# awslabs/palace

Hardware: AMD Instinct MI355X
Metric: curl-curl Mult DOF/s + PCG iters/s, p=3 H(curl) 10M DOF @1/2/4/8 GPU (higher is better)
Workload: dtype f64

## Files before the change

palace_amd/csrc/pa_internal.hpp:

```cpp
#pragma once

#include <hip/hip_runtime.h>

#include <cstdint>
#include <cstdio>
#include <stdexcept>
#include <string>
#include <vector>

#include "../../include/palace_amd.h"
#include "pa_stream_host.hpp"

struct pa_op;
typedef struct pa_op pa_op_fwd;

struct pa_csr {
  bool symmetric = true;
  int32_t nrows = 0;
  int32_t ncols = 0;
  int64_t nnz = 0;
  int32_t *d_rowptr = nullptr, *d_col = nullptr;
  double *d_val = nullptr;
};

// ... 128 lines not shown
  int32_t *d_lidx = nullptr;
  int32_t *d_sidx = nullptr;
  int32_t *d_sidx_bc = nullptr;
  uint16_t *d_perm = nullptr;
  uint16_t *d_perm_x = nullptr;
  int32_t *d_shared = nullptr;
  int32_t *d_shared_bc = nullptr;
  std::vector<int32_t> h_shared;
  std::vector<char> h_price_skip;
  int n_shared = 0;
  std::vector<uint16_t> h_perm;
  std::vector<int32_t> h_sidx;
  double *d_ye = nullptr;
  double *d_ye2 = nullptr;
  int32_t *d_tptr = nullptr;
  int32_t *d_tent = nullptr;
  uint32_t *d_idxc = nullptr;
  bool stream_default = true;
  uint32_t *d_perm_s_bc = nullptr;
  std::vector<uint32_t> h_perm_s;
  int32_t *d_rhdr_bc = nullptr, *d_rpos_bc = nullptr;
  int n_shared_bc = 0;
  uint32_t *d_perm_s = nullptr;
  uint32_t *d_flagw = nullptr, *d_flagw_bc = nullptr, *d_slots = nullptr;
  int n_slot_patterns = 0;
  double *d_coef_s = nullptr;
  int32_t *d_rhdr = nullptr, *d_rpos = nullptr;
  int n_runs = 0, n_runs_bc = 0;
  uint32_t *d_rchunk = nullptr, *d_rchunk_bc = nullptr;
  uint32_t *d_flagw_all = nullptr, *d_rchunk_all = nullptr;
  uint32_t *d_perm_s_all = nullptr;
  int32_t *d_rhdr_all = nullptr, *d_rpos_all = nullptr;
  int n_all = 0, n_runs_all = 0;
  std::vector<char> h_ess_flag;
  std::vector<double> Bc, Gc, Bo;
  double *d_tab = nullptr;
  bool iso = false;
  std::vector<uint8_t> ctx_blob;
  CoeffHost c0, c1;
};

struct DenseSub {
  Geom *geom = nullptr;
  int fe_type = 0, P = 0, Q = 0, Qpad = 0, nch = 0, ne = 0, nb = 0, lsize = 0, KP = 0, PT = 0;
  int qf = 0, mode = 0;
  bool contra = false;
  bool ye_rows = false;
// ... 187 lines not shown
```

palace_amd/csrc/pa_nd_hex_stream.hip:

```cpp
#include <algorithm>
#include <map>

#include "pa_nd_hex_core.hpp"

#ifndef PA_CPLX_QAHEAD
#define PA_CPLX_QAHEAD 0
#endif
#ifndef PA_STREAM_QAHEAD
#define PA_STREAM_QAHEAD 0
#endif
#ifndef PA_KM_MINW_LOW
#define PA_KM_MINW_LOW 2
#endif
#ifndef PA_KM_MINW
#define PA_KM_MINW 2
#endif

namespace pa {

typedef double d2v __attribute__((ext_vector_type(2)));

#ifdef PA_STREAM_TRACE
constexpr int kTraceWG = 64, kTraceBatches = 14, kTraceStamps = 12;
__device__ unsigned long long g_trace[kTraceWG * kTraceBatches * kTraceStamps];
#define PA_STAMP(k)                                                                                          \
  do {                                                                                                       \
    if (tr_on && tr_b < kTraceBatches && lane == 0)                                                          \
      g_trace[((size_t)blockIdx.x * kTraceBatches + tr_b) * kTraceStamps + (k)] = __builtin_readcyclecounter(); \
  } while (0)
#else
#define PA_STAMP(k) \
  do {              \
  } while (0)
#endif

#ifdef PA_STREAM_OLD_LDS
__host__ __device__ constexpr int stream_lds_elem(const int raw) { return raw; }
#else
__host__ __device__ constexpr int stream_lds_elem(const int raw) { return (raw + 15) / 32 * 32 + 16; }
#endif

template <int P1>
struct NDStreamArgs {
  int ne, nbatch, chunk;
  const uint32_t *idxc;
  const uint32_t *flagw;
  const uint32_t *slots;
  const double *qdata;
  const double *qaff;
  double wq2[2];
  const double *coef;
  const double *xn, *gtab;
  const double *x;
  double *y, *ye;
  const double *x1, *coef1;
  double *y1, *ye1;
  const double *qdata1;
  int qm[2], qc[2], qn[2];
  int nsplit;
  const double *xg0, *xg1;
  const unsigned long long *xg_sel;
  double *yg;
  NDTab<P1, 4> tab;
};

template <int P1, bool USE_U, bool USE_C, bool METRIC, int MINW, int GPOS, bool CPLX = false, bool SPLIT = false, int GEOMN = 0>
__global__ __launch_bounds__(64 * kWavesPerBlock, MINW) void nd_hex_stream_kernel(const NDStreamArgs<P1> a) {
  static_assert(!CPLX || (USE_U && USE_C), "the complex form is built on the curl-curl + mass kernels");
  static_assert(!(CPLX && SPLIT), "no split-vector form of the complex kernel");
  static_assert(!GEOMN || (!USE_U && USE_C && !METRIC && !CPLX), "geometry from the nodes: the curl-curl kernel");
  constexpr int Q1 = 4;
  constexpr bool AFF = (!CPLX || METRIC) && !GEOMN && !(PA_STREAM_QAHEAD && MINW == 2);
#ifdef PA_STREAM_EARLY
  constexpr bool EARLY_IDX = true;
#else
  constexpr bool EARLY_IDX = P1 < 3;
#endif
  using L = typename std::conditional<P1 == 3 && !CPLX && USE_C && !USE_U, NDLayoutInPlaceSwz3, NDLayout<P1, Q1>>::type;
  constexpr int NC = P1 + 1, PP = 3 * P1 * NC * NC, NPL = (PP + 15) / 16, NPK = (NPL + 3) / 4;
#ifdef PA_METRIC6
  constexpr int NG = METRIC ? 6 : 6 * ((USE_U ? 1 : 0) + (USE_C ? 1 : 0));
#else
  constexpr int NG = METRIC ? (USE_U ? 7 : 6) : 6 * ((USE_U ? 1 : 0) + (USE_C ? 1 : 0));
#endif
  static_assert(PP <= 256, "8-bit slots");
  using streamhost::kIdxPattern;
  using streamhost::kIdxStart0;
  using streamhost::kIdxWords;
  constexpr int LDS_SIDE = (PP + 1) / 2 + (NPK + 1) * 8;
  constexpr int LDS_XN = GEOMN ? 82 : 0;
  constexpr int LDS_ELEM = stream_lds_elem(L::ELEM_PAD + LDS_SIDE + 12 + LDS_XN);
  extern __shared__ __attribute__((aligned(16))) double smem[];
  const int lane = threadIdx.x & 63;
  const int wave = __builtin_amdgcn_readfirstlane(threadIdx.x >> 6);
  const int xcd = blockIdx.x & 7;
  const int base = xcd * a.chunk, bend = min(base + a.chunk, a.nbatch);
  const int stride = (int)(gridDim.x >> 3) * kWavesPerBlock;
  int b = base + (int)(blockIdx.x >> 3) * kWavesPerBlock + wave;
  if (b >= bend) return;
  const double *xsel = (CPLX && ((lane >> 4) & 1)) ? a.x1 : a.x;
  const double *xgh = nullptr;
  if (SPLIT) xgh = ((a.xg_sel ? *a.xg_sel : 0ull) & 1ull) ? a.xg1 : a.xg0;
  auto load_idx = [&](const int bb, const int sub, const int t, int (&s)[NPL + 2], unsigned (&p)[NPK + 1]) {
    const int e = CPLX ? bb * 2 + (sub >> 1) : bb * 4 + sub;
    const uint32_t *ic = a.idxc + (size_t)e * kIdxWords;
#pragma unroll
    for (int r = 0; r < NPL; r++) s[r] = (int)__builtin_nontemporal_load(&ic[r]);
    s[NPL] = (int)__builtin_nontemporal_load(&ic[kIdxStart0 + t]);
    s[NPL + 1] = (int)__builtin_nontemporal_load(&ic[kIdxStart0 + 16 + (t & 3)]);
    p[NPK] = __builtin_nontemporal_load(&a.flagw[(size_t)e * 16 + t]);
    p[0] = __builtin_nontemporal_load(&ic[kIdxPattern]);
  };
  auto gather = [&](int (&s)[NPL + 2], unsigned (&p)[NPK + 1], double (&xv)[NPL], int *stab, const int t) {
    stab[t] = s[NPL];
    if (t < 4) stab[16 + t] = s[NPL + 1];
    wave_sync();
    const unsigned fw = p[NPK];
    {
      const uint32_t *sl = a.slots + (size_t)p[0] * (NPK * 16) + t;
#pragma unroll
      for (int k = 0; k < NPK; k++) p[k] = sl[16 * k];
    }
#pragma unroll
    for (int r = 0; r < NPL; r++) {
      const unsigned w = (unsigned)s[r], low = (w & 0xffffu) & ((2u << t) - 1u);
      const int rid = (int)((w >> 16) & 31u) + __popc(low) - 1;
      const int pos = low ? 16 * r + 31 - __clz((int)low) : (int)((w >> 21) & 255u);
      int dof = stab[rid] + (t + 16 * r - pos);
      if (!(16 * r + 15 < PP) && t + 16 * r >= PP) dof = 0;
      xv[r] = SPLIT ? (dof < a.nsplit ? xsel : xgh)[dof] : xsel[dof];
      const int word = dof | ((fw >> (2 * r + 1)) & 1u ? kExclBit : 0) | ((fw >> (18 + r)) & 1u ? kEssBit : 0);
      s[r] = (fw >> (2 * r)) & 1u ? -1 - word : word;
    }
  };
  auto settle = [&](unsigned (&p)[NPK + 1]) { asm volatile("" : "+v"(p[NPK])); };
  int sA[NPL + 2];
  unsigned pA[NPK + 1];
  double xv[NPL];
  load_idx(b, lane >> 4, lane & 15, sA, pA);
  gather(sA, pA, xv,
         reinterpret_cast<int *>(smem + (size_t)(wave * 4 + (lane >> 4)) * LDS_ELEM + L::ELEM_PAD + LDS_SIDE), lane & 15);
#pragma unroll
  for (int r = 0; r < NPL; r++) asm volatile("" : "+v"(xv[r]));
  settle(pA);

  constexpr bool QAHEAD = PA_STREAM_QAHEAD && MINW == 2 && (!CPLX || (PA_CPLX_QAHEAD && !METRIC));
  d2v gq[GEOMN ? 1 : 2 * NG];
  double xl[GEOMN ? 6 : 1];
  auto load_xn = [&](const int ee, const int t) {
    const double *xp = a.xn + (size_t)ee * 81;
#pragma unroll
    for (int r = 0; r < (GEOMN ? 6 : 1); r++) xl[r] = (t + 16 * r < 81) ? __builtin_nontemporal_load(&xp[t + 16 * r]) : 0.0;
  };
  auto load_q = [&](const int ee, const int t, const int aff) {
    if (GEOMN) return load_xn(ee, t);
    if (AFF && !(CPLX && !METRIC)) {
      constexpr int NS = METRIC ? 7 : NG;
      const int rs = aff ? 1 : 16;
      const d2v *g = aff ? reinterpret_cast<const d2v *>(a.qaff) + (size_t)ee * (2 * NS)
                         : reinterpret_cast<const d2v *>(a.qdata) + ((size_t)ee * (2 * NS * 16) + t);
#pragma unroll
      for (int k = 0; k < 2 * NG; k++) gq[k] = __builtin_nontemporal_load(&g[rs * k]);
      return;
    }
    if (CPLX && !METRIC) {
      const int grp = (lane >> 4) & 1;
      const int mo = a.qm[grp], co = a.qc[grp];
// ... 23 lines not shown
    PA_STAMP(0);
    int lo = lane;
    asm volatile("" : "+v"(lo));
    const int sub = lo >> 4, t = lo & 15, ta = t & 3, tb = t >> 2;
    double *sm = smem + (size_t)(wave * 4 + sub) * LDS_ELEM;
    int *side = reinterpret_cast<int *>(sm + L::ELEM_PAD);
    int *stab = side + 2 * LDS_SIDE;
#ifdef PA_STREAM_OLD_LDS
    const int lx = L::parity_xor(sub);
#else
    constexpr int lx = 0;
#endif
    const int e = CPLX ? b * 2 + (sub >> 1) : b * 4 + sub;

    const int aff = AFF ? __builtin_amdgcn_readfirstlane((int)(pA[NPK] >> 31)) : 0;
    if (!QAHEAD) load_q(e, t, aff);
    d2v ce = {0.0, 0.0}, ci = {0.0, 0.0};
    if (METRIC || GEOMN) ce = reinterpret_cast<const d2v *>(a.coef)[e];
    if (CPLX && METRIC) ci = reinterpret_cast<const d2v *>(a.coef1)[e];

#pragma unroll
    for (int r = 0; r < NPL; r++) {
      if (16 * r + 15 < PP || t + 16 * r < PP) {
        const int sv = sA[r], df = sv >= 0 ? sv : -1 - sv;
        const double v = (df & kEssBit) ? 0.0 : xv[r];
        sm[(pA[r >> 2] >> (8 * (r & 3))) & 255u] = sv >= 0 ? v : -v;
        side[t + 16 * r] = sv;
      }
    }
#pragma unroll
    for (int k = 0; k <= NPK; k++) side[2 * ((PP + 1) / 2) + 16 * k + t] = (int)pA[k];
    PA_STAMP(1);
    wave_sync();
    double uin[3][NC];
#pragma unroll
    for (int C = 0; C < 3; C++) {
      const int ni = (C == 0) ? P1 : NC, nj = (C == 1) ? P1 : NC, nk = (C == 2) ? P1 : NC;
      const bool act = ta < nj && tb < nk;
#pragma unroll
      for (int i = 0; i < NC; i++) uin[C][i] = (act && i < ni) ? sm[C * P1 * NC * NC + i + ni * (ta + nj * tb)] : 0.0;
    }
    wave_sync();

    const int kn = b + stride;
    const bool more = kn < bend;
    const int bn = more ? kn : b;
    int sB[NPL + 2];
    unsigned pB[NPK + 1];
    if (EARLY_IDX) {
      load_idx(bn, sub, t, sB, pB);
      __builtin_amdgcn_sched_barrier(0);
    }
    PA_STAMP(2);
    double U[3][Q1], CU[3][Q1];
#pragma unroll
    for (int c = 0; c < 3; c++)
#pragma unroll
      for (int q = 0; q < Q1; q++) U[c][q] = 0.0, CU[c][q] = 0.0;
    nd_fwd_comp<0, P1, Q1, USE_U, USE_C, L>(a, e, true, true, ta, tb, lx, sm, uin[0], U, CU);
    nd_fwd_comp<1, P1, Q1, USE_U, USE_C, L>(a, e, true, true, ta, tb, lx, sm, uin[1], U, CU);
    nd_fwd_comp<2, P1, Q1, USE_U, USE_C, L>(a, e, true, true, ta, tb, lx, sm, uin[2], U, CU);

    PA_STAMP(3);
    PA_STAMP(4);
    if (!EARLY_IDX) {
      __builtin_amdgcn_sched_barrier(0);
      load_idx(bn, sub, t, sB, pB);
      __builtin_amdgcn_sched_barrier(0);
    }

    constexpr bool PARK = GEOMN == 2;
    double Pz[GEOMN ? 3 : 1][3][PARK ? 1 : 3];
    double Pl = 0.0;
    double cw = 0.0;
    double *xs = sm + L::ELEM_PAD + LDS_SIDE + 12;
    auto park = [&](const int q) -> double * { return (q < 12 ? sm + 16 * q : xs + 16 * (q - 12)) + t; };
    if (GEOMN) {
#pragma unroll
      for (int r = 0; r < 6; r++)
        if (t + 16 * r < 81) xs[t + 16 * r] = xl[r];
      wave_sync();
      const double *gt = a.gtab;
      double bx[3], gx[3], by[3], gy[3];
#pragma unroll
      for (int i = 0; i < 3; i++) bx[i] = gt[ta * 3 + i], gx[i] = gt[12 + ta * 3 + i], by[i] = gt[tb * 3 + i], gy[i] = gt[12 + tb * 3 + i];
      cw = ce[1] * gt[24 + ta] * gt[24 + tb];
#pragma unroll
      for (int k = 0; k < 3; k++) {
        double acc[3][3];
#pragma unroll
// ... 132 lines not shown
        if (AFF) {
#pragma unroll
          for (int c = 0; c < 3; c++) {
            if (USE_U) U[c][qz] *= wab;
            if (USE_C) CU[c][qz] *= wab;
          }
        }
      }
    }

    if (GEOMN == 2) wave_sync();
    PA_STAMP(5);

    if (QAHEAD) {
      __builtin_amdgcn_sched_barrier(0);
      load_q(CPLX ? bn * 2 + (sub >> 1) : bn * 4 + sub, t, 0);
      __builtin_amdgcn_sched_barrier(0);
    }
    double xB[NPL];
    nd_bwd_comp<0, P1, Q1, USE_U, USE_C, L>(a, e, true, true, ta, tb, lx, sm, uin[0], U, CU);
    PA_STAMP(6);
    if (GPOS == 1) {
      __builtin_amdgcn_sched_barrier(0);
      gather(sB, pB, xB, stab, t);
      settle(pB);
      __builtin_amdgcn_sched_barrier(0);
    }
    PA_STAMP(7);
    nd_bwd_comp<1, P1, Q1, USE_U, USE_C, L>(a, e, true, true, ta, tb, lx, sm, uin[1], U, CU);
    if (GPOS == 2) {
      __builtin_amdgcn_sched_barrier(0);
      gather(sB, pB, xB, stab, t);
      settle(pB);
      __builtin_amdgcn_sched_barrier(0);
    }
    nd_bwd_comp<2, P1, Q1, USE_U, USE_C, L>(a, e, true, true, ta, tb, lx, sm, uin[2], U, CU);

    PA_STAMP(8);
#pragma unroll
    for (int C = 0; C < 3; C++) {
      const int ni = (C == 0) ? P1 : NC, nj = (C == 1) ? P1 : NC, nk = (C == 2) ? P1 : NC;
      const bool act = ta < nj && tb < nk;
#pragma unroll
      for (int i = 0; i < NC; i++)
        if (act && i < ni) sm[C * P1 * NC * NC + i + ni * (ta + nj * tb)] = uin[C][i];
    }
    wave_sync();
#pragma unroll
    for (int r = 0; r < NPL; r++) {
      const int m = (16 * r + 15 < PP) ? t + 16 * r : min(t + 16 * r, PP - 1), mt = m & 15, mr = m >> 4;
      const unsigned fl = (unsigned)side[2 * ((PP + 1) / 2) + 16 * NPK + mt] >> (2 * mr);
      const double v = sm[((unsigned)side[2 * ((PP + 1) / 2) + 16 * (mr >> 2) + mt] >> (8 * (mr & 3))) & 255u];
      const int sv = side[m], df = sv >= 0 ? sv : -1 - sv, d = df & (kExclBit - 1);
      double *yd = (CPLX && (sub & 1)) ? a.y1 : a.y;
      if (SPLIT) yd = d < a.nsplit ? a.y : a.yg;
      double *dst = (fl & 2u) ? yd + d : ((CPLX && (sub & 1)) ? a.ye1 : a.ye) + ((size_t)e * PP + m);
      *dst = (fl & 1u) ? -v : v;
    }
    wave_sync();
    PA_STAMP(9);
#ifdef PA_STREAM_TRACE
    tr_b++;
#endif
    if (!more) break;
    b = bn;
#pragma unroll
    for (int r = 0; r < NPL; r++) sA[r] = sB[r], xv[r] = xB[r];
#pragma unroll
    for (int k = 0; k <= NPK; k++) pA[k] = pB[k];
  }
}

using streamhost::RunHdr;
using streamhost::RunChunk;

constexpr int kGatherILP = 4;
struct GatherPart2 {
  const double *ye1, *x1;
  double *y1;
};
template <bool STEP, bool DUAL = false>
__global__ __launch_bounds__(256) void et_run_gather_kernel_t(const int n, const RunChunk *__restrict__ chunk,
                                                              const RunHdr *__restrict__ hdr, const int32_t *__restrict__ rpos,
                                                              const double *__restrict__ ye, double *__restrict__ y,
                                                              const int accumulate, const double *__restrict__ x,
                                                              const int ess_policy, const int nsplit, double *__restrict__ yg,
                                                              const GatherStep st, const GatherPart2 p2) {
  const int k0 = blockIdx.x * (256 * kGatherILP) + threadIdx.x;
  const int lane = threadIdx.x & 63;
  RunHdr h[kGatherILP];
  int pe[kGatherILP], d[kGatherILP], j[kGatherILP], run[kGatherILP];
  bool live[kGatherILP], fix[kGatherILP];
// ... 242 lines not shown
      const size_t e = k / P;
      const int m = (int)(k - e * P), t = m & 15, r = m >> 4;
      pp[(e * (npk + 1) + npk) * 16 + t] |= 2u << (2 * r);
      dropped += so.h_price_skip[k] ? 1 : 0, freed += so.h_price_skip[k] ? 0 : 1;
    }
    std::vector<int32_t> shared2;
    for (int d = 0; d < so.lsize; d++)
      if (cnt2[d] > 1) shared2.push_back(d);
    fprintf(stderr, "PALACE_AMD_PRICE_BLOCK=%d: %zu of %zu E-vector entries dropped, %zu more leave the gather; shared dofs %zu -> %zu\n",
            price_group, dropped, nnz, freed, so.h_shared.size(), shared2.size());
    so.h_shared = shared2;
    so.n_shared = (int)shared2.size();
  }
  if (so.fe_type == PA_FE_HCURL && !wide_form(so)) {
    stream_affine_setup(so);
    const int npl = (P + 15) / 16, npk = (npl + 3) / 4;
    for (size_t b = 0; b < so.qd->batch_aff.size(); b++)
      if (so.qd->batch_aff[b])
        for (size_t e = 4 * b; e < 4 * b + 4; e++)
          for (int t = 0; t < 16; t++) pp[(e * (npk + 1) + npk) * 16 + t] |= streamhost::kAffBit;
  }
  so.h_perm_s = pp;
  if (so.fe_type == PA_FE_HCURL && !wide_form(so)) {
    const int npl = (P + 15) / 16, npk = (npl + 3) / 4, nep = (ne + 3) & ~3, sw = npk * 16;
    std::vector<uint32_t> flagw((size_t)nep * 16), slots;
    std::map<std::vector<uint32_t>, uint32_t> dict;
    std::vector<uint32_t> key((size_t)sw);
    for (int e = 0; e < nep; e++) {
      const uint32_t *row = &pp[(size_t)e * (npk + 1) * 16];
      std::copy(row + sw, row + sw + 16, flagw.begin() + (size_t)e * 16);
      key.assign(row, row + sw);
      auto it = dict.find(key);
      if (it == dict.end()) {
        it = dict.emplace(key, (uint32_t)dict.size()).first;
        slots.insert(slots.end(), key.begin(), key.end());
      }
      ic[(size_t)e * streamhost::kIdxWords + streamhost::kIdxPattern] = it->second;
    }
    so.n_slot_patterns = (int)dict.size();
    so.d_flagw = dev_upload(flagw.data(), flagw.size());
    so.d_slots = dev_upload(slots.data(), slots.size());
  }
  so.d_idxc = dev_upload(ic.data(), ic.size());
  so.d_perm_s = dev_upload(pp.data(), pp.size());
  if (so.qd->metric || (so.iso && so.qf == PA_QF_HDIV_33 && so.geom->d_xnodes)) stream_element_coefficients(so);

  std::vector<uint32_t> code;
  std::vector<RunHdr> hdr;
  std::vector<int32_t> rpos;
  streamhost::build_runs(ne, P, so.lsize, so.h_sidx.data(), so.h_shared, code, hdr, rpos, nullptr,
                         so.h_price_skip.empty() ? nullptr : so.h_price_skip.data());
  {
    const std::vector<RunChunk> ch = streamhost::run_chunks(code);
    so.d_rchunk = dev_upload(reinterpret_cast<const uint32_t *>(ch.data()), 4 * ch.size());
  }
  so.d_rhdr = dev_upload(reinterpret_cast<const int32_t *>(hdr.data()), 2 * hdr.size());
  so.d_rpos = dev_upload(rpos.data(), rpos.size());
  so.n_runs = (int)hdr.size() - 1;
}

void stream_set_essential(SubOp &so, const std::vector<char> &flag) {
  if (!so.d_idxc) return;
  so.h_ess_flag = flag;
  if (so.n_all > 0) {
// ... 6 lines not shown
  const bool wide = wide_form(so);
  const int npkw = ((P + 31) / 32 + 1) / 2;
  for (size_t k = 0; k < nnz; k++) {
    if (flag[streamhost::dof_of(so.h_sidx[k])]) {
      const size_t e = k / P;
      if (wide) {
        const int m = (int)(k - e * P), t = m & 31, r = m >> 5;
        uint32_t &w = pb[(e * npkw + (r >> 1)) * 32 + t];
        w &= ~(streamhost::kWideExcl << (16 * (r & 1)));
        w |= streamhost::kWideEss << (16 * (r & 1));
        continue;
      }
      const int m = (int)(k - e * P), t = m & 15, r = m >> 4;
      uint32_t &fw = pb[(e * (npk + 1) + npk) * 16 + t];
      fw &= ~(2u << (2 * r));
      fw |= 1u << (18 + r);
    }
  }
  hipFree(so.d_perm_s_bc);
  so.d_perm_s_bc = dev_upload(pb.data(), pb.size());
  if (so.d_flagw) {
    const int nep = (so.ne + 3) & ~3;
    std::vector<uint32_t> fb((size_t)nep * 16);
    for (int e = 0; e < nep; e++) std::copy(&pb[((size_t)e * (npk + 1) + npk) * 16], &pb[((size_t)e * (npk + 1) + npk) * 16] + 16, fb.begin() + (size_t)e * 16);
    hipFree(so.d_flagw_bc);
    so.d_flagw_bc = dev_upload(fb.data(), fb.size());
  }
  std::vector<int32_t> count((size_t)so.lsize, 0);
  for (size_t k = 0; k < nnz; k++) count[streamhost::dof_of(so.h_sidx[k])]++;
  std::vector<int32_t> shared;
  shared.reserve(so.h_shared.size());
  if (!so.h_price_skip.empty()) {
    std::fill(count.begin(), count.end(), 0);
    for (size_t k = 0; k < nnz; k++)
      if (!so.h_price_skip[k]) count[streamhost::dof_of(so.h_sidx[k])]++;
  }
  for (int d = 0; d < so.lsize; d++)
    if (count[d] != 1 || flag[d]) shared.push_back(d);
  std::vector<uint32_t> code;
  std::vector<RunHdr> hdr;
  std::vector<int32_t> rpos;
  streamhost::build_runs(so.ne, P, so.lsize, so.h_sidx.data(), shared, code, hdr, rpos, flag.data(),
                         so.h_price_skip.empty() ? nullptr : so.h_price_skip.data());
  hipFree(so.d_rhdr_bc), hipFree(so.d_rpos_bc), hipFree(so.d_rchunk_bc);
  {
    const std::vector<RunChunk> ch = streamhost::run_chunks(code);
    so.d_rchunk_bc = dev_upload(reinterpret_cast<const uint32_t *>(ch.data()), 4 * ch.size());
  }
  so.d_rhdr_bc = dev_upload(reinterpret_cast<const int32_t *>(hdr.data()), 2 * hdr.size());
  so.d_rpos_bc = dev_upload(rpos.data(), rpos.size());
  so.n_shared_bc = (int)shared.size();
  so.n_runs_bc = (int)hdr.size() - 1;
}

void free_stream(SubOp &so) {
  hipFree(so.d_idxc), hipFree(so.d_perm_s), hipFree(so.d_perm_s_bc), hipFree(so.d_coef_s);
  hipFree(so.d_flagw), hipFree(so.d_flagw_bc), hipFree(so.d_slots);
  hipFree(so.d_flagw_all), hipFree(so.d_perm_s_all), hipFree(so.d_rchunk_all), hipFree(so.d_rhdr_all), hipFree(so.d_rpos_all);
  so.d_flagw_all = so.d_perm_s_all = nullptr, so.d_rchunk_all = nullptr, so.d_rhdr_all = so.d_rpos_all = nullptr, so.n_all = 0;
  hipFree(so.d_rhdr), hipFree(so.d_rpos), hipFree(so.d_rhdr_bc), hipFree(so.d_rpos_bc), hipFree(so.d_rchunk), hipFree(so.d_rchunk_bc);
}

static int device_cus() {
  static int cus = [] {
    int dev = 0, n = 0;
    if (hipGetDevice(&dev) != hipSuccess || hipDeviceGetAttribute(&n, hipDeviceAttributeMultiprocessorCount, dev) != hipSuccess || n <= 0)
      n = 256;
    return n;
  }();
  return cus;
}

template <int P1, bool U, bool C, bool METRIC, int MINW, int GPOS, bool CPLX = false, bool SPLIT = false, int GEOMN = 0>
static void launch_gpos(const SubOp &so, NDStreamArgs<P1> &a, hipStream_t s) {
  using L = typename std::conditional<P1 == 3 && !CPLX && C && !U, NDLayoutInPlaceSwz3, NDLayout<P1, 4>>::type;
  for (int i = 0; i < HalfTab<P1, 4>::LEN; i++) a.tab.Bo[i] = so.Bo[i];
  for (int i = 0; i < HalfTab<P1 + 1, 4>::LEN; i++) a.tab.Bc[i] = so.Bc[i], a.tab.Gc[i] = so.Gc[i];
  constexpr int PP = 3 * P1 * (P1 + 1) * (P1 + 1);
  constexpr int NPK = ((PP + 15) / 16 + 3) / 4;
  const size_t lds = sizeof(double) * (size_t)(kWavesPerBlock * 4) *
                     stream_lds_elem(L::ELEM_PAD + (PP + 1) / 2 + (NPK + 1) * 8 + 12 + (GEOMN ? 82 : 0));
  static const int wg_env = getenv("PALACE_AMD_STREAM_WG") ? atoi(getenv("PALACE_AMD_STREAM_WG")) : 0;
  static const int per_cu_query = [&] {
    int nb = 0;
    if (hipOccupancyMaxActiveBlocksPerMultiprocessor(&nb, nd_hex_stream_kernel<P1, U, C, METRIC, MINW, GPOS, CPLX, SPLIT, GEOMN>,
                                                     64 * kWavesPerBlock, lds) != hipSuccess || nb <= 0)
      nb = 8;
    return std::min({nb, MINW * 4 / kWavesPerBlock, (int)(160 * 1024 / lds), 8});
  }();
  const int per_cu = wg_env > 0 ? wg_env : per_cu_query;
  const int per_xcd = std::max(1, device_cus() / 8) * per_cu;
  if (CPLX) a.nbatch = (so.ne + 1) / 2;
  else a.nbatch = (so.ne + 3) / 4;
  if (a.nbatch == 0) return;
  a.chunk = (a.nbatch + 7) / 8;
  const int waves = std::min(per_xcd * kWavesPerBlock, a.chunk);
  const int wgx = std::max(1, (waves + kWavesPerBlock - 1) / kWavesPerBlock);
  hipLaunchKernelGGL((nd_hex_stream_kernel<P1, U, C, METRIC, MINW, GPOS, CPLX, SPLIT, GEOMN>), dim3(8 * wgx), dim3(64 * kWavesPerBlock),
                     lds, s, a);
  PA_HIP(hipGetLastError());
}

template <int P1, bool U, bool C, bool METRIC, int MINW_>
static void launch_variant(const SubOp &so, NDStreamArgs<P1> &a, hipStream_t s) {
#ifdef PA_STREAM_MINW2
  constexpr int MINW = 2;
#else
  constexpr int MINW = MINW_;
#endif
  constexpr int GPOS = U ? 2 : 1;
  if (a.nsplit >= 0)
    return launch_gpos<P1, U, C, METRIC, MINW, GPOS, false, true>(so, a, s);
  launch_gpos<P1, U, C, METRIC, MINW, GPOS>(so, a, s);
}

template <int P1>
static void launch_p(const SubOp &so, const double *x, double *y, bool masked, hipStream_t s, const SplitIO *split,
                     bool all = false) {
  NDStreamArgs<P1> a{};
  a.nsplit = -1, a.xg0 = a.xg1 = nullptr, a.xg_sel = nullptr, a.yg = nullptr;
  if (split) {
    PA_REQUIRE(split->n_true >= 0 && split->n_true <= so.lsize, "split point outside the local vector");
    a.nsplit = split->n_true;
    a.xg0 = split->xg0 - split->n_true, a.xg1 = (split->xg1 ? split->xg1 : split->xg0) - split->n_true;
    a.xg_sel = split->sel, a.yg = split->yg - split->n_true;
  }
  a.ne = so.ne, a.nbatch = 0;
  a.idxc = so.d_idxc;
  a.flagw = all ? so.d_flagw_all : (masked ? so.d_flagw_bc : so.d_flagw);
  a.slots = so.d_slots;
  a.qdata = so.qd->d;
  a.qaff = so.qd->d_aff, a.wq2[0] = so.qd->wq2[0], a.wq2[1] = so.qd->wq2[1];
#ifdef PA_METRIC6
  if (so.geom->w1.size() == 4) a.wq2[0] = so.geom->w1[0], a.wq2[1] = so.geom->w1[1];
#endif
  a.coef = so.d_coef_s;
  a.xn = nullptr, a.gtab = nullptr;
  a.x = x, a.y = y, a.ye = so.d_ye;
  const bool m = so.qd->metric;
  switch (so.qf) {
    case PA_QF_HDIV_33: {
      const char *ge = getenv("PALACE_AMD_STREAM_GEOM");
      const bool geomn = ge && std::string(ge) == "nodes";
      if (!m && geomn && P1 == 3 && so.iso && so.geom->d_xnodes && so.d_coef_s && !split) {
        a.xn = so.geom->d_xnodes, a.gtab = so.geom->d_gtab;
        const char *ve = getenv("PALACE_AMD_GEOMN_VARIANT");
        if (ve && std::string(ve) == "w2g2") launch_gpos<P1, false, true, false, 2, 2, false, false, (P1 == 3 ? 1 : 0)>(so, a, s);
        else if (ve && std::string(ve) == "park3g1") launch_gpos<P1, false, true, false, 3, 1, false, false, (P1 == 3 ? 2 : 0)>(so, a, s);
        else if (ve && std::string(ve) == "park3g2") launch_gpos<P1, false, true, false, 3, 2, false, false, (P1 == 3 ? 2 : 0)>(so, a, s);
        else launch_gpos<P1, false, true, false, 2, 1, false, false, (P1 == 3 ? 1 : 0)>(so, a, s);
        break;
      }
      if (m) launch_variant<P1, false, true, true, (P1 == 3 ? 2 : 3)>(so, a, s); else launch_variant<P1, false, true, false, 3>(so, a, s);
// ... 43 lines not shown
  };
  if (!enabled || !qf_ok(sr) || !qf_ok(si)) return false;
  if (sr.geom != si.geom || sr.ne != si.ne || sr.p != si.p || sr.P != si.P || sr.q1d != si.q1d) return false;
  auto iso_ok = [](const SubOp &so) {
    return so.iso && ((so.q1d == 4 && so.p <= 3) || (so.q1d == 5 && so.p <= 4 && nd_hex_stream5_ok(so))) && !so.geom->h_attr.empty();
  };
  const bool metric = iso_ok(sr) && iso_ok(si) && sr.d_idxc && sr.d_coef_s && sr.qd && sr.qd->metric;
  auto packed_ok = [](const SubOp &so) {
    return ((so.q1d == 4 && so.p <= 3) || (so.q1d == 5 && so.p <= 4 && nd_hex_stream5_ok(so))) && so.qd && !so.qd->metric &&
           so.qd->ncomp == (so.qf == PA_QF_HDIVMASS_33 ? 12 : 6);
  };
  const bool packed = packed_ok(sr) && packed_ok(si) && sr.d_idxc;
  if (!metric && !packed) return false;
  return sr.h_sidx == si.h_sidx;
}

template <int P1>
static void launch_complex_p(const SubOp &sr, const SubOp &si, const double *xr, const double *xi, double *yr, double *yi,
                             double *ye_i, bool masked, hipStream_t s) {
  NDStreamArgs<P1> a{};
  a.ne = sr.ne, a.nbatch = 0;
  a.idxc = sr.d_idxc;
  a.flagw = masked ? sr.d_flagw_bc : sr.d_flagw;
  a.slots = sr.d_slots;
  a.qdata = sr.qd->d;
  if (sr.qd->metric) a.qaff = sr.qd->d_aff, a.wq2[0] = sr.qd->wq2[0], a.wq2[1] = sr.qd->wq2[1];
  a.coef = sr.d_coef_s, a.coef1 = si.d_coef_s;
  a.xn = nullptr, a.gtab = nullptr;
  a.x = xr, a.x1 = xi, a.y = yr, a.y1 = yi, a.ye = sr.d_ye, a.ye1 = ye_i;
  a.nsplit = -1, a.xg0 = a.xg1 = nullptr, a.xg_sel = nullptr, a.yg = nullptr;
  a.qdata1 = nullptr;
  if (sr.qd->metric) return launch_gpos<P1, true, true, true, 2, 2, true>(sr, a, s);
  const SubOp *ops[2] = {&sr, &si};
  for (int g = 0; g < 2; g++) {
    const int qf = ops[g]->qf;
    a.qn[g] = ops[g]->qd->ncomp;
    a.qm[g] = (qf == PA_QF_HCURL_33 || qf == PA_QF_HDIVMASS_33) ? 0 : -1;
    a.qc[g] = qf == PA_QF_HDIV_33 ? 0 : (qf == PA_QF_HDIVMASS_33 ? 6 : -1);
  }
  a.qdata1 = si.qd->d;
  launch_gpos<P1, true, true, false, 2, 2, true>(sr, a, s);
}

void launch_nd_hex_stream_complex(const SubOp &sr, const SubOp &si, const double *xr, const double *xi, double *yr, double *yi,
                                  double *ye_i, bool masked, hipStream_t s) {
  if (sr.q1d == 5) return launch_nd_hex_stream5_complex(sr, si, xr, xi, yr, yi, ye_i, masked, s);
  switch (sr.p) {
// ... 70 lines not shown
        fw[(e * (npk + 1) + npk) * 16 + t] |= 1u << (18 + r);
      } else {
        const int m = (int)(k - e * P), t = m & 15, r = m >> 4;
        fw[e * 16 + t] |= 1u << (18 + r);
      }
    }
  }
  std::vector<int32_t> all;
  all.reserve((size_t)so.lsize);
  for (int d = 0; d < so.lsize; d++)
    if (present[d] || flag[d]) all.push_back(d);
  if ((int)all.size() != so.lsize) return false;
  std::vector<uint32_t> code;
  std::vector<RunHdr> hdr;
  std::vector<int32_t> rpos;
  streamhost::build_runs(so.ne, P, so.lsize, so.h_sidx.data(), all, code, hdr, rpos, flag.data(), nullptr);
  const std::vector<RunChunk> ch = streamhost::run_chunks(code);
  so.d_rchunk_all = dev_upload(reinterpret_cast<const uint32_t *>(ch.data()), 4 * ch.size());
  so.d_rhdr_all = dev_upload(reinterpret_cast<const int32_t *>(hdr.data()), 2 * hdr.size());
  so.d_rpos_all = dev_upload(rpos.data(), rpos.size());
  so.n_all = (int)all.size(), so.n_runs_all = (int)hdr.size() - 1;
  if (wide || h1)
    so.d_perm_s_all = dev_upload(fw.data(), fw.size());
  else
    so.d_flagw_all = dev_upload(fw.data(), fw.size());
  return true;
}

void launch_et_run_gather_step(const SubOp &so, const double *x, const GatherStep &step, int ess_policy, hipStream_t s,
                               const SplitIO *split) {
  PA_REQUIRE(so.n_all > 0, "stream_build_all has not been called");
  PA_REQUIRE(!split || (step.iface_mask && step.t_iface), "split form of the fused step: interface mask and buffer missing");
  const int n = so.n_all;
  hipLaunchKernelGGL(et_run_gather_kernel_t<true>, dim3((n + 256 * kGatherILP - 1) / (256 * kGatherILP)), dim3(256), 0, s, n,
                     reinterpret_cast<const RunChunk *>(so.d_rchunk_all), reinterpret_cast<const RunHdr *>(so.d_rhdr_all), so.d_rpos_all,
                     so.d_ye, nullptr, 0, x, ess_policy, split ? split->n_true : 0x7fffffff, split ? split->yg - split->n_true : nullptr,
                     step, GatherPart2{});
  PA_HIP(hipGetLastError());
}

#ifdef PA_STREAM_TRACE
}
extern "C" int pa_debug_stream_trace(unsigned long long *out, int n) {
  const int total = pa::kTraceWG * pa::kTraceBatches * pa::kTraceStamps;
  if (n < total) return -total;
  if (hipMemcpyFromSymbol(out, HIP_SYMBOL(pa::g_trace), sizeof(unsigned long long) * total) != hipSuccess) return -1;
  return total;
}
// ... 4 lines not shown
```

palace_amd/csrc/pa_stream_host.hpp:

```cpp
#pragma once

#include <cstdint>
#include <stdexcept>
#include <vector>

namespace pa {

constexpr int kEssBit = 1 << 30;
constexpr int kExclBit = 1 << 29;

namespace streamhost {

struct RunHdr {
  uint32_t dof0;
  int32_t ptr;
};
constexpr uint32_t kRunDofMask = (1u << 27) - 1u;
inline int run_dof0(const RunHdr &h) { return (int)(h.dof0 & kRunDofMask); }
inline int run_len(const RunHdr &h) { return (int)((h.dof0 >> 27) & 15u) + 1; }
inline bool run_ess(const RunHdr &h) { return (h.dof0 >> 31) != 0; }

inline int dof_of(int32_t s) { return s >= 0 ? s : -1 - s; }

constexpr int kIdxWords = 32, kIdxStart0 = 12, kIdxMaxRuns = kIdxWords - kIdxStart0, kIdxStart0H1 = 4;
constexpr int kIdxPattern = 11;
constexpr uint32_t kAffBit = 1u << 31;

inline int index_dof(const uint32_t *ic, int m, int start0 = kIdxStart0) {
  const int r = m >> 4, t = m & 15;
  const uint32_t w = ic[r], low = (w & 0xffffu) & ((2u << t) - 1u);
  int bits = 0, top = -1;
  for (int j = 0; j < 16; j++)
    if (low >> j & 1u) bits++, top = j;
  const int rid = (int)((w >> 16) & 31u) + bits - 1;
  if (rid < 0 || rid >= kIdxWords - start0) throw std::runtime_error("index decode: entry without a run");
  const int pos = low ? 16 * r + top : (int)((w >> 21) & 255u);
  return (int)ic[start0 + rid] + (m - pos);
}

inline bool pack_index(int ne, int P, int lsize, const int32_t *sidx, const uint16_t *perm, std::vector<uint32_t> &ic,
                       std::vector<uint32_t> &pp, int start0 = kIdxStart0) {
  if (P > 256) throw std::runtime_error("element too large for 8-bit slots");
  if (lsize >= kExclBit) throw std::runtime_error("too many local dofs for the streaming index encoding");
  const int nep = (ne + 3) & ~3, npl = (P + 15) / 16, npk = (npl + 3) / 4;
  if (npl > 9 || npl > start0) throw std::runtime_error("element too large for the flag word / slice words");
  const int max_runs = kIdxWords - start0;
  const size_t nnz = (size_t)ne * P;
  std::vector<int32_t> count((size_t)lsize, 0);
  for (size_t k = 0; k < nnz; k++) count[dof_of(sidx[k])]++;
  ic.assign((size_t)nep * kIdxWords, 0u);
  pp.assign((size_t)nep * (npk + 1) * 16, 0u);
  for (int e = 0; e < nep; e++) {
    uint32_t *ice = &ic[(size_t)e * kIdxWords];
    if (e >= ne) {
      ice[0] = 1u;
      for (int r = 1; r < npl; r++) ice[r] = 1u << 16;
      continue;
    }
    int nruns = 0, lastpos = 0, prev = -2;
    for (int m = 0; m < P; m++) {
// ... 165 lines not shown
      if (extend)
        for (int c = 0; c < nc; c++)
          if (step[hdr.back().ptr + c] == 0) step[hdr.back().ptr + c] = (int8_t)(tk[tptr[d] + c] % P - k0[hdr.back().ptr + c] % P);
    }
    if (!extend) {
      hdr.push_back(RunHdr{(uint32_t)d, (int32_t)rpos.size()});
      for (int c = 0; c < nc; c++) {
        const int k = tk[tptr[d] + c];
        k0.push_back(k), step.push_back(0);
        rpos.push_back((uint32_t)position(k / P, k % P) | ((orients && orients[k]) ? kDenseRunNeg : 0u));
      }
      len = 0;
    }
    if (hdr.size() >= (1u << 27)) throw std::runtime_error("too many runs for the gather code");
    code[(size_t)d] = (uint32_t)(hdr.size() - 1) << 4 | (uint32_t)len;
    hdr.back().dof0 = (hdr.back().dof0 & ~(15u << 27)) | ((uint32_t)len << 27);
    len++;
  }
  for (size_t i = 0; i < rpos.size(); i++)
    if (step[i] < 0) rpos[i] |= kDenseRunBack;
  hdr.push_back(RunHdr{0u, (int32_t)rpos.size()});
}

}
}
```

Before: 65.51 billion.

## Precompute per-pattern DOF decode tables and repack flag words for sign-flip XOR

The in-kernel index decoding (popc/clz run lookup on packed index words) is replaced by a host-built per-pattern table. The table holds each slot's run id and offset, so the gather becomes a table load plus an add. Flag words are re-encoded to three bits per row and merged into the DOF word, which turns sign handling into an XOR on the high bits of the double and drops one LDS side row. The pattern id now comes from a separate array and is prefetched one batch ahead. In exchange, the pattern dictionary keys now include the index words, so there may be more distinct patterns and a larger table competing for cache.

```diff
diff --git a/palace_amd/csrc/pa_internal.hpp b/palace_amd/csrc/pa_internal.hpp
--- a/palace_amd/csrc/pa_internal.hpp
+++ b/palace_amd/csrc/pa_internal.hpp
@@ -174,7 +174,7 @@
   int32_t *d_rhdr_bc = nullptr, *d_rpos_bc = nullptr;
   int n_shared_bc = 0;
   uint32_t *d_perm_s = nullptr;
-  uint32_t *d_flagw = nullptr, *d_flagw_bc = nullptr, *d_slots = nullptr;
+  uint32_t *d_flagw = nullptr, *d_flagw_bc = nullptr, *d_slots = nullptr, *d_pattern = nullptr;
   int n_slot_patterns = 0;
   double *d_coef_s = nullptr;
   int32_t *d_rhdr = nullptr, *d_rpos = nullptr;
diff --git a/palace_amd/csrc/pa_nd_hex_stream.hip b/palace_amd/csrc/pa_nd_hex_stream.hip
--- a/palace_amd/csrc/pa_nd_hex_stream.hip
+++ b/palace_amd/csrc/pa_nd_hex_stream.hip
@@ -1,5 +1,4 @@
 #include <algorithm>
-#include <map>
 
 #include "pa_nd_hex_core.hpp"
 
@@ -46,6 +45,7 @@
   const uint32_t *idxc;
   const uint32_t *flagw;
   const uint32_t *slots;
+  const uint32_t *pattern;
   const double *qdata;
   const double *qaff;
   double wq2[2];
@@ -77,17 +77,16 @@
   constexpr bool EARLY_IDX = P1 < 3;
 #endif
   using L = typename std::conditional<P1 == 3 && !CPLX && USE_C && !USE_U, NDLayoutInPlaceSwz3, NDLayout<P1, Q1>>::type;
-  constexpr int NC = P1 + 1, PP = 3 * P1 * NC * NC, NPL = (PP + 15) / 16, NPK = (NPL + 3) / 4;
+  constexpr int NC = P1 + 1, PP = 3 * P1 * NC * NC, NPL = (PP + 15) / 16, NPK = (NPL + 3) / 4, NPH = (NPL + 1) / 2;
 #ifdef PA_METRIC6
   constexpr int NG = METRIC ? 6 : 6 * ((USE_U ? 1 : 0) + (USE_C ? 1 : 0));
 #else
   constexpr int NG = METRIC ? (USE_U ? 7 : 6) : 6 * ((USE_U ? 1 : 0) + (USE_C ? 1 : 0));
 #endif
   static_assert(PP <= 256, "8-bit slots");
-  using streamhost::kIdxPattern;
   using streamhost::kIdxStart0;
   using streamhost::kIdxWords;
-  constexpr int LDS_SIDE = (PP + 1) / 2 + (NPK + 1) * 8;
+  constexpr int LDS_SIDE = (PP + 1) / 2 + NPK * 8;
   constexpr int LDS_XN = GEOMN ? 82 : 0;
   constexpr int LDS_ELEM = stream_lds_elem(L::ELEM_PAD + LDS_SIDE + 12 + LDS_XN);
   extern __shared__ __attribute__((aligned(16))) double smem[];
@@ -101,48 +100,57 @@
   const double *xsel = (CPLX && ((lane >> 4) & 1)) ? a.x1 : a.x;
   const double *xgh = nullptr;
   if (SPLIT) xgh = ((a.xg_sel ? *a.xg_sel : 0ull) & 1ull) ? a.xg1 : a.xg0;
-  auto load_idx = [&](const int bb, const int sub, const int t, int (&s)[NPL + 2], unsigned (&p)[NPK + 1]) {
-    const int e = CPLX ? bb * 2 + (sub >> 1) : bb * 4 + sub;
+  auto elem_of = [&](const int bb, const int sub) { return CPLX ? bb * 2 + (sub >> 1) : bb * 4 + sub; };
+  auto load_pattern = [&](const int bb, const int sub) { return __builtin_nontemporal_load(&a.pattern[elem_of(bb, sub)]); };
+  auto load_idx = [&](const int bb, const int bnx, const unsigned pat, const int sub, const int t, int (&s)[NPH + 2],
+                      unsigned (&p)[NPK + 1], unsigned &pn) {
+    const int e = elem_of(bb, sub);
     const uint32_t *ic = a.idxc + (size_t)e * kIdxWords;
-#pragma unroll
-    for (int r = 0; r < NPL; r++) s[r] = (int)__builtin_nontemporal_load(&ic[r]);
-    s[NPL] = (int)__builtin_nontemporal_load(&ic[kIdxStart0 + t]);
-    s[NPL + 1] = (int)__builtin_nontemporal_load(&ic[kIdxStart0 + 16 + (t & 3)]);
+    const uint32_t *dt = a.slots + (size_t)pat * ((NPK + NPH) * 16) + (NPK * 16 + t);
+#pragma unroll
+    for (int k = 0; k < NPH; k++) s[k] = (int)dt[16 * k];
+    s[NPH] = (int)__builtin_nontemporal_load(&ic[kIdxStart0 + t]);
+    s[NPH + 1] = (int)__builtin_nontemporal_load(&ic[kIdxStart0 + 16 + (t & 3)]);
     p[NPK] = __builtin_nontemporal_load(&a.flagw[(size_t)e * 16 + t]);
-    p[0] = __builtin_nontemporal_load(&ic[kIdxPattern]);
+    p[0] = pat;
+    pn = load_pattern(bnx, sub);
   };
-  auto gather = [&](int (&s)[NPL + 2], unsigned (&p)[NPK + 1], double (&xv)[NPL], int *stab, const int t) {
-    stab[t] = s[NPL];
-    if (t < 4) stab[16 + t] = s[NPL + 1];
+  auto gather = [&](const int (&s)[NPH + 2], unsigned (&p)[NPK + 1], int (&w)[NPL], double (&xv)[NPL], int *stab, const int t) {
+    stab[t] = s[NPH];
+    if (t < 4) stab[16 + t] = s[NPH + 1];
     wave_sync();
     const unsigned fw = p[NPK];
     {
-      const uint32_t *sl = a.slots + (size_t)p[0] * (NPK * 16) + t;
+      const uint32_t *sl = a.slots + (size_t)p[0] * ((NPK + NPH) * 16) + t;
 #pragma unroll
       for (int k = 0; k < NPK; k++) p[k] = sl[16 * k];
     }
 #pragma unroll
     for (int r = 0; r < NPL; r++) {
-      const unsigned w = (unsigned)s[r], low = (w & 0xffffu) & ((2u << t) - 1u);
-      const int rid = (int)((w >> 16) & 31u) + __popc(low) - 1;
-      const int pos = low ? 16 * r + 31 - __clz((int)low) : (int)((w >> 21) & 255u);
-      int dof = stab[rid] + (t + 16 * r - pos);
-      if (!(16 * r + 15 < PP) && t + 16 * r >= PP) dof = 0;
+      const unsigned h = (unsigned)s[r >> 1];
+      const unsigned rid = (r & 1) ? (h >> 16) & 31u : h & 31u, off = (r & 1) ? h >> 21 : (h >> 5) & 2047u;
+      const int dof = stab[rid] + (int)off;
       xv[r] = SPLIT ? (dof < a.nsplit ? xsel : xgh)[dof] : xsel[dof];
-      const int word = dof | ((fw >> (2 * r + 1)) & 1u ? kExclBit : 0) | ((fw >> (18 + r)) & 1u ? kEssBit : 0);
-      s[r] = (fw >> (2 * r)) & 1u ? -1 - word : word;
+      w[r] = dof | (int)((fw >> (3 * r)) << 29);
     }
   };
-  auto settle = [&](unsigned (&p)[NPK + 1]) { asm volatile("" : "+v"(p[NPK])); };
-  int sA[NPL + 2];
+  auto settle = [&](unsigned (&p)[NPK + 1], unsigned &pn) { asm volatile("" : "+v"(p[NPK]), "+v"(pn)); };
+  auto flip_by = [](const double v, const unsigned w) {
+    return __hiloint2double(__double2hiint(v) ^ (int)(w & streamhost::kFlipBit), __double2loint(v));
+  };
+  int sA[NPL];
   unsigned pA[NPK + 1];
   double xv[NPL];
-  load_idx(b, lane >> 4, lane & 15, sA, pA);
-  gather(sA, pA, xv,
-         reinterpret_cast<int *>(smem + (size_t)(wave * 4 + (lane >> 4)) * LDS_ELEM + L::ELEM_PAD + LDS_SIDE), lane & 15);
+  unsigned patn;
+  {
+    const int sub = lane >> 4, kn0 = b + stride;
+    int s0[NPH + 2];
+    load_idx(b, kn0 < bend ? kn0 : b, load_pattern(b, sub), sub, lane & 15, s0, pA, patn);
+    gather(s0, pA, sA, xv, reinterpret_cast<int *>(smem + (size_t)(wave * 4 + sub) * LDS_ELEM + L::ELEM_PAD + LDS_SIDE), lane & 15);
+  }
 #pragma unroll
   for (int r = 0; r < NPL; r++) asm volatile("" : "+v"(xv[r]));
-  settle(pA);
+  settle(pA, patn);
 
   constexpr bool QAHEAD = PA_STREAM_QAHEAD && MINW == 2 && (!CPLX || (PA_CPLX_QAHEAD && !METRIC));
   d2v gq[GEOMN ? 1 : 2 * NG];
@@ -212,14 +220,14 @@
 #pragma unroll
     for (int r = 0; r < NPL; r++) {
       if (16 * r + 15 < PP || t + 16 * r < PP) {
-        const int sv = sA[r], df = sv >= 0 ? sv : -1 - sv;
-        const double v = (df & kEssBit) ? 0.0 : xv[r];
-        sm[(pA[r >> 2] >> (8 * (r & 3))) & 255u] = sv >= 0 ? v : -v;
+        const int sv = sA[r];
+        const double v = (sv & kEssBit) ? 0.0 : xv[r];
+        sm[(pA[r >> 2] >> (8 * (r & 3))) & 255u] = flip_by(v, (unsigned)sv);
         side[t + 16 * r] = sv;
       }
     }
 #pragma unroll
-    for (int k = 0; k <= NPK; k++) side[2 * ((PP + 1) / 2) + 16 * k + t] = (int)pA[k];
+    for (int k = 0; k < NPK; k++) side[2 * ((PP + 1) / 2) + 16 * k + t] = (int)pA[k];
     PA_STAMP(1);
     wave_sync();
     double uin[3][NC];
@@ -234,11 +242,11 @@
 
     const int kn = b + stride;
     const bool more = kn < bend;
-    const int bn = more ? kn : b;
-    int sB[NPL + 2];
-    unsigned pB[NPK + 1];
+    const int bn = more ? kn : b, bnn = kn + stride < bend ? kn + stride : bn;
+    int sB[NPH + 2], wB[NPL];
+    unsigned pB[NPK + 1], patnn;
     if (EARLY_IDX) {
-      load_idx(bn, sub, t, sB, pB);
+      load_idx(bn, bnn, patn, sub, t, sB, pB, patnn);
       __builtin_amdgcn_sched_barrier(0);
     }
     PA_STAMP(2);
@@ -255,7 +263,7 @@
     PA_STAMP(4);
     if (!EARLY_IDX) {
       __builtin_amdgcn_sched_barrier(0);
-      load_idx(bn, sub, t, sB, pB);
+      load_idx(bn, bnn, patn, sub, t, sB, pB, patnn);
       __builtin_amdgcn_sched_barrier(0);
     }
 
@@ -434,16 +442,16 @@
     PA_STAMP(6);
     if (GPOS == 1) {
       __builtin_amdgcn_sched_barrier(0);
-      gather(sB, pB, xB, stab, t);
-      settle(pB);
+      gather(sB, pB, wB, xB, stab, t);
+      settle(pB, patnn);
       __builtin_amdgcn_sched_barrier(0);
     }
     PA_STAMP(7);
     nd_bwd_comp<1, P1, Q1, USE_U, USE_C, L>(a, e, true, true, ta, tb, lx, sm, uin[1], U, CU);
     if (GPOS == 2) {
       __builtin_amdgcn_sched_barrier(0);
-      gather(sB, pB, xB, stab, t);
-      settle(pB);
+      gather(sB, pB, wB, xB, stab, t);
+      settle(pB, patnn);
       __builtin_amdgcn_sched_barrier(0);
     }
     nd_bwd_comp<2, P1, Q1, USE_U, USE_C, L>(a, e, true, true, ta, tb, lx, sm, uin[2], U, CU);
@@ -461,13 +469,12 @@
 #pragma unroll
     for (int r = 0; r < NPL; r++) {
       const int m = (16 * r + 15 < PP) ? t + 16 * r : min(t + 16 * r, PP - 1), mt = m & 15, mr = m >> 4;
-      const unsigned fl = (unsigned)side[2 * ((PP + 1) / 2) + 16 * NPK + mt] >> (2 * mr);
       const double v = sm[((unsigned)side[2 * ((PP + 1) / 2) + 16 * (mr >> 2) + mt] >> (8 * (mr & 3))) & 255u];
-      const int sv = side[m], df = sv >= 0 ? sv : -1 - sv, d = df & (kExclBit - 1);
+      const unsigned sv = (unsigned)side[m], d = sv & (unsigned)(kExclBit - 1);
       double *yd = (CPLX && (sub & 1)) ? a.y1 : a.y;
-      if (SPLIT) yd = d < a.nsplit ? a.y : a.yg;
-      double *dst = (fl & 2u) ? yd + d : ((CPLX && (sub & 1)) ? a.ye1 : a.ye) + ((size_t)e * PP + m);
-      *dst = (fl & 1u) ? -v : v;
+      if (SPLIT) yd = (int)d < a.nsplit ? a.y : a.yg;
+      double *dst = (sv & (unsigned)kExclBit) ? yd + d : ((CPLX && (sub & 1)) ? a.ye1 : a.ye) + ((size_t)e * PP + m);
+      *dst = flip_by(v, sv);
     }
     wave_sync();
     PA_STAMP(9);
@@ -477,9 +484,10 @@
     if (!more) break;
     b = bn;
 #pragma unroll
-    for (int r = 0; r < NPL; r++) sA[r] = sB[r], xv[r] = xB[r];
+    for (int r = 0; r < NPL; r++) sA[r] = wB[r], xv[r] = xB[r];
 #pragma unroll
     for (int k = 0; k <= NPK; k++) pA[k] = pB[k];
+    patn = patnn;
   }
 }
 
@@ -768,24 +776,14 @@
   }
   so.h_perm_s = pp;
   if (so.fe_type == PA_FE_HCURL && !wide_form(so)) {
-    const int npl = (P + 15) / 16, npk = (npl + 3) / 4, nep = (ne + 3) & ~3, sw = npk * 16;
-    std::vector<uint32_t> flagw((size_t)nep * 16), slots;
-    std::map<std::vector<uint32_t>, uint32_t> dict;
-    std::vector<uint32_t> key((size_t)sw);
-    for (int e = 0; e < nep; e++) {
-      const uint32_t *row = &pp[(size_t)e * (npk + 1) * 16];
-      std::copy(row + sw, row + sw + 16, flagw.begin() + (size_t)e * 16);
-      key.assign(row, row + sw);
-      auto it = dict.find(key);
-      if (it == dict.end()) {
-        it = dict.emplace(key, (uint32_t)dict.size()).first;
-        slots.insert(slots.end(), key.begin(), key.end());
-      }
-      ic[(size_t)e * streamhost::kIdxWords + streamhost::kIdxPattern] = it->second;
-    }
-    so.n_slot_patterns = (int)dict.size();
+    const int npl = (P + 15) / 16, npk = (npl + 3) / 4, nep = (ne + 3) & ~3;
+    std::vector<uint32_t> flagw((size_t)nep * 16), table, pattern;
+    for (int e = 0; e < nep; e++)
+      for (int t = 0; t < 16; t++) flagw[(size_t)e * 16 + t] = streamhost::device_flag_word(pp[((size_t)e * (npk + 1) + npk) * 16 + t], npl);
+    so.n_slot_patterns = streamhost::build_patterns(nep, P, ic, pp, table, pattern);
     so.d_flagw = dev_upload(flagw.data(), flagw.size());
-    so.d_slots = dev_upload(slots.data(), slots.size());
+    so.d_slots = dev_upload(table.data(), table.size());
+    so.d_pattern = dev_upload(pattern.data(), pattern.size());
   }
   so.d_idxc = dev_upload(ic.data(), ic.size());
   so.d_perm_s = dev_upload(pp.data(), pp.size());
@@ -838,7 +836,8 @@
   if (so.d_flagw) {
     const int nep = (so.ne + 3) & ~3;
     std::vector<uint32_t> fb((size_t)nep * 16);
-    for (int e = 0; e < nep; e++) std::copy(&pb[((size_t)e * (npk + 1) + npk) * 16], &pb[((size_t)e * (npk + 1) + npk) * 16] + 16, fb.begin() + (size_t)e * 16);
+    for (int e = 0; e < nep; e++)
+      for (int t = 0; t < 16; t++) fb[(size_t)e * 16 + t] = streamhost::device_flag_word(pb[((size_t)e * (npk + 1) + npk) * 16 + t], npl);
     hipFree(so.d_flagw_bc);
     so.d_flagw_bc = dev_upload(fb.data(), fb.size());
   }
@@ -871,7 +870,7 @@
 
 void free_stream(SubOp &so) {
   hipFree(so.d_idxc), hipFree(so.d_perm_s), hipFree(so.d_perm_s_bc), hipFree(so.d_coef_s);
-  hipFree(so.d_flagw), hipFree(so.d_flagw_bc), hipFree(so.d_slots);
+  hipFree(so.d_flagw), hipFree(so.d_flagw_bc), hipFree(so.d_slots), hipFree(so.d_pattern);
   hipFree(so.d_flagw_all), hipFree(so.d_perm_s_all), hipFree(so.d_rchunk_all), hipFree(so.d_rhdr_all), hipFree(so.d_rpos_all);
   so.d_flagw_all = so.d_perm_s_all = nullptr, so.d_rchunk_all = nullptr, so.d_rhdr_all = so.d_rpos_all = nullptr, so.n_all = 0;
   hipFree(so.d_rhdr), hipFree(so.d_rpos), hipFree(so.d_rhdr_bc), hipFree(so.d_rpos_bc), hipFree(so.d_rchunk), hipFree(so.d_rchunk_bc);
@@ -895,7 +894,7 @@
   constexpr int PP = 3 * P1 * (P1 + 1) * (P1 + 1);
   constexpr int NPK = ((PP + 15) / 16 + 3) / 4;
   const size_t lds = sizeof(double) * (size_t)(kWavesPerBlock * 4) *
-                     stream_lds_elem(L::ELEM_PAD + (PP + 1) / 2 + (NPK + 1) * 8 + 12 + (GEOMN ? 82 : 0));
+                     stream_lds_elem(L::ELEM_PAD + (PP + 1) / 2 + NPK * 8 + 12 + (GEOMN ? 82 : 0));
   static const int wg_env = getenv("PALACE_AMD_STREAM_WG") ? atoi(getenv("PALACE_AMD_STREAM_WG")) : 0;
   static const int per_cu_query = [&] {
     int nb = 0;
@@ -911,7 +910,8 @@
   if (a.nbatch == 0) return;
   a.chunk = (a.nbatch + 7) / 8;
   const int waves = std::min(per_xcd * kWavesPerBlock, a.chunk);
-  const int wgx = std::max(1, (waves + kWavesPerBlock - 1) / kWavesPerBlock);
+  int wgx = std::max(1, (waves + kWavesPerBlock - 1) / kWavesPerBlock);
+  if (const char *cap = getenv("PALACE_AMD_STREAM_WGX")) wgx = std::max(1, std::min(wgx, atoi(cap)));
   hipLaunchKernelGGL((nd_hex_stream_kernel<P1, U, C, METRIC, MINW, GPOS, CPLX, SPLIT, GEOMN>), dim3(8 * wgx), dim3(64 * kWavesPerBlock),
                      lds, s, a);
   PA_HIP(hipGetLastError());
@@ -944,7 +944,7 @@
   a.ne = so.ne, a.nbatch = 0;
   a.idxc = so.d_idxc;
   a.flagw = all ? so.d_flagw_all : (masked ? so.d_flagw_bc : so.d_flagw);
-  a.slots = so.d_slots;
+  a.slots = so.d_slots, a.pattern = so.d_pattern;
   a.qdata = so.qd->d;
   a.qaff = so.qd->d_aff, a.wq2[0] = so.qd->wq2[0], a.wq2[1] = so.qd->wq2[1];
 #ifdef PA_METRIC6
@@ -1034,7 +1034,7 @@
   a.ne = sr.ne, a.nbatch = 0;
   a.idxc = sr.d_idxc;
   a.flagw = masked ? sr.d_flagw_bc : sr.d_flagw;
-  a.slots = sr.d_slots;
+  a.slots = sr.d_slots, a.pattern = sr.d_pattern;
   a.qdata = sr.qd->d;
   if (sr.qd->metric) a.qaff = sr.qd->d_aff, a.wq2[0] = sr.qd->wq2[0], a.wq2[1] = sr.qd->wq2[1];
   a.coef = sr.d_coef_s, a.coef1 = si.d_coef_s;
@@ -1151,8 +1151,10 @@
   so.n_all = (int)all.size(), so.n_runs_all = (int)hdr.size() - 1;
   if (wide || h1)
     so.d_perm_s_all = dev_upload(fw.data(), fw.size());
-  else
+  else {
+    for (uint32_t &w : fw) w = streamhost::device_flag_word(w, npl);
     so.d_flagw_all = dev_upload(fw.data(), fw.size());
+  }
   return true;
 }
 
diff --git a/palace_amd/csrc/pa_stream_host.hpp b/palace_amd/csrc/pa_stream_host.hpp
--- a/palace_amd/csrc/pa_stream_host.hpp
+++ b/palace_amd/csrc/pa_stream_host.hpp
@@ -1,6 +1,7 @@
 #pragma once
 
 #include <cstdint>
+#include <map>
 #include <stdexcept>
 #include <vector>
 
@@ -26,16 +27,70 @@
 constexpr int kIdxPattern = 11;
 constexpr uint32_t kAffBit = 1u << 31;
 
-inline int index_dof(const uint32_t *ic, int m, int start0 = kIdxStart0) {
+inline void index_run(const uint32_t *ic, int m, int &rid, int &pos, int start0 = kIdxStart0) {
   const int r = m >> 4, t = m & 15;
   const uint32_t w = ic[r], low = (w & 0xffffu) & ((2u << t) - 1u);
   int bits = 0, top = -1;
   for (int j = 0; j < 16; j++)
     if (low >> j & 1u) bits++, top = j;
-  const int rid = (int)((w >> 16) & 31u) + bits - 1;
+  rid = (int)((w >> 16) & 31u) + bits - 1;
   if (rid < 0 || rid >= kIdxWords - start0) throw std::runtime_error("index decode: entry without a run");
-  const int pos = low ? 16 * r + top : (int)((w >> 21) & 255u);
+  pos = low ? 16 * r + top : (int)((w >> 21) & 255u);
+}
+inline int index_dof(const uint32_t *ic, int m, int start0 = kIdxStart0) {
+  int rid, pos;
+  index_run(ic, m, rid, pos, start0);
   return (int)ic[start0 + rid] + (m - pos);
+}
+
+constexpr int kDecRunBits = 5;
+inline uint32_t decode_half(const uint32_t *ic, int m) {
+  int rid, pos;
+  index_run(ic, m, rid, pos, kIdxStart0);
+  return (uint32_t)rid | (uint32_t)(m - pos) << kDecRunBits;
+}
+inline int decode_rows(int P) { return ((P + 15) / 16 + 1) / 2; }
+inline void pack_decode(const uint32_t *ic, int P, uint32_t *rows) {
+  for (int k = 0; k < decode_rows(P) * 16; k++) rows[k] = 0u;
+  for (int m = 0; m < P; m++) {
+    const int r = m >> 4, t = m & 15;
+    rows[(r >> 1) * 16 + t] |= decode_half(ic, m) << (16 * (r & 1));
+  }
+}
+inline int table_dof(const uint32_t *rows, const uint32_t *ic, int m) {
+  const int r = m >> 4, t = m & 15;
+  const uint32_t h = (rows[(r >> 1) * 16 + t] >> (16 * (r & 1))) & 0xffffu;
+  return (int)ic[kIdxStart0 + (h & ((1u << kDecRunBits) - 1u))] + (int)(h >> kDecRunBits);
+}
+inline int build_patterns(int nep, int P, std::vector<uint32_t> &ic, const std::vector<uint32_t> &pp, std::vector<uint32_t> &table,
+                          std::vector<uint32_t> &pattern) {
+  const int npl = (P + 15) / 16, npk = (npl + 3) / 4, sw = npk * 16, dw = decode_rows(P) * 16;
+  std::map<std::vector<uint32_t>, uint32_t> dict;
+  std::vector<uint32_t> key, dec((size_t)dw);
+  table.clear();
+  pattern.assign((size_t)nep, 0u);
+  for (int e = 0; e < nep; e++) {
+    const uint32_t *row = &pp[(size_t)e * (npk + 1) * 16];
+    uint32_t *ice = &ic[(size_t)e * kIdxWords];
+    key.assign(row, row + sw);
+    key.insert(key.end(), ice, ice + npl);
+    auto it = dict.find(key);
+    if (it == dict.end()) {
+      it = dict.emplace(key, (uint32_t)dict.size()).first;
+      pack_decode(ice, P, dec.data());
+      table.insert(table.end(), row, row + sw);
+      table.insert(table.end(), dec.begin(), dec.end());
+    }
+    ice[kIdxPattern] = pattern[(size_t)e] = it->second;
+  }
+  return (int)dict.size();
+}
+constexpr uint32_t kFlipBit = 1u << 31;
+inline uint32_t device_flag_word(uint32_t fw, int npl) {
+  uint32_t out = fw & kAffBit;
+  for (int r = 0; r < npl; r++)
+    out |= ((fw >> (2 * r + 1)) & 1u) << (3 * r) | ((fw >> (18 + r)) & 1u) << (3 * r + 1) | ((fw >> (2 * r)) & 1u) << (3 * r + 2);
+  return out;
 }
 
 inline bool pack_index(int ne, int P, int lsize, const int32_t *sidx, const uint16_t *perm, std::vector<uint32_t> &ic,
@@ -247,5 +302,11 @@
   hdr.push_back(RunHdr{0u, (int32_t)rpos.size()});
 }
 
-}
-}
+inline uint32_t device_index_word(const uint32_t *table, int P, uint32_t pat, const uint32_t *ic, const uint32_t *flagw, int m) {
+  const int npl = (P + 15) / 16, npk = (npl + 3) / 4, rows = npk + decode_rows(P);
+  const uint32_t dof = (uint32_t)table_dof(table + ((size_t)pat * rows + npk) * 16, ic, m);
+  return dof | (flagw[m & 15] >> (3 * (m >> 4))) << 29;
+}
+
+}
+}
```

After: 66.85 billion (median of 6 runs). 1.02x the previous value.
